# leejaeyong7/tiny-cuda-nn

Measured on AMD Instinct MI355X. Metric: training_step throughput (samples/s) HashGrid+64-wide FFMLP, batch=256k; % fp16-MFMA peak, higher is better.
Workload: dtype f16

## Files before the change

include/tcnn_amd.h:

```cpp
#ifndef TCNN_AMD_H
#define TCNN_AMD_H

#include <stddef.h>
#include <stdint.h>

#ifdef __cplusplus
extern "C" {
#endif

#define TCNN_OK 0
#define TCNN_ERROR 1

#define TCNN_PRECISION_FP32 0
#define TCNN_PRECISION_FP16 1

#define TCNN_GRADIENT_IGNORE 0
#define TCNN_GRADIENT_OVERWRITE 1
#define TCNN_GRADIENT_ACCUMULATE 2

#define TCNN_LAYOUT_SOA 0
#define TCNN_LAYOUT_AOS 1

#define TCNN_LOG_INFO 0
#define TCNN_LOG_DEBUG 1
// ... 91 lines not shown
int      tcnn_trainer_initialize_params(tcnn_trainer_t t);
int      tcnn_trainer_update_hyperparams(tcnn_trainer_t t, const char* json);
const char* tcnn_trainer_hyperparams(tcnn_trainer_t t);
int      tcnn_trainer_serialize(tcnn_trainer_t t, int serialize_optimizer, const void** out_bytes, size_t* out_size);
int      tcnn_trainer_deserialize(tcnn_trainer_t t, const void* bytes, size_t size);
const char* tcnn_trainer_network_hyperparams(tcnn_trainer_t t);
uint32_t tcnn_trainer_optimizer_step_count(tcnn_trainer_t t);
int  tcnn_trainer_profile_next_step(tcnn_trainer_t t);
int  tcnn_trainer_profile_collect(tcnn_trainer_t t, tcnn_stream_t stream, float* ms_per_piece , uint32_t* n_steps);
size_t tcnn_trainer_params_updated_in_flush(tcnn_trainer_t t);
size_t tcnn_trainer_image_preps(tcnn_trainer_t t);
size_t tcnn_trainer_scatter_wide_fallbacks(tcnn_trainer_t t);
size_t tcnn_trainer_optimizer_prologue_steps(tcnn_trainer_t t);
size_t tcnn_trainer_list_scatters(tcnn_trainer_t t);
size_t tcnn_module_list_scatters(tcnn_module_t m);
const char* tcnn_trainer_last_step_kernel(tcnn_trainer_t t);

int   tcnn_module_set_max_level(tcnn_module_t m, float max_level);
float tcnn_module_max_level(tcnn_module_t m);
int   tcnn_module_set_max_level_gpu(tcnn_module_t m, const float* per_sample);
int   tcnn_trainer_set_max_level(tcnn_trainer_t t, float max_level);
int   tcnn_trainer_set_max_level_gpu(tcnn_trainer_t t, const float* per_sample);
float tcnn_trainer_max_level(tcnn_trainer_t t);
int tcnn_train_ctx_keeps_weight_gradient_slabs(tcnn_trainer_t t, tcnn_train_ctx_t ctx);


int         tcnn_module_layer_sizes(tcnn_module_t m, uint32_t* rows_cols, size_t capacity, size_t* n_layers_out);
int         tcnn_optimizer_create(const char* optimizer_json, size_t n_params, const uint32_t* layer_sizes, size_t n_layers, tcnn_optimizer_t* out);
void        tcnn_optimizer_destroy(tcnn_optimizer_t o);
int         tcnn_optimizer_step(tcnn_optimizer_t o, tcnn_stream_t stream, float loss_scale, float* params_full_precision, void* params_half,
// ... 17 lines not shown
```

tiny-cuda-nn_amd/csrc/capi.cpp:

```cpp
#include "../../include/tcnn_amd.h"

#include "model.h"

#include <mutex>
#include <string>

using namespace tcnn_amd;

namespace {
thread_local std::string g_last_error;
tcnn_amd::Switches g_switches;
std::mutex g_switches_mutex;

bool env_is(const char* name, char c) {
	const char* e = getenv(name);
	return e && e[0] == c;
}
int env_01(const char* name) {
	const char* e = getenv(name);
	return (e && (e[0] == '0' || e[0] == '1')) ? e[0] - '0' : -1;
}

template <typename F>
int guarded(F&& f) {
// ... 61 lines not shown
	w.fused_step = !env_is("TCNN_AMD_FUSED_STEP", '0');
	w.side_jobs = !env_is("TCNN_AMD_SIDE_JOBS", '0');
	w.live_image = !env_is("TCNN_AMD_LIVE_IMAGE", '0');
	w.adam_steps32 = env_is("TCNN_AMD_ADAM_STEPS32", '1');
#ifdef TCNN_AMD_DEV
	w.adam_in_flush = env_is("TCNN_AMD_ADAM_IN_FLUSH", '1');
#endif
	w.adam_in_reduce = !env_is("TCNN_AMD_ADAM_IN_REDUCE", '0');
	w.adam_prologue = !env_is("TCNN_AMD_ADAM_PROLOGUE", '0');
	w.adam_prologue_refused = env_is("TCNN_AMD_ADAM_PROLOGUE", 'r');
	w.mlp_r32 = !env_is("TCNN_AMD_MLP_R32", '0');
	w.mlp_r32a = env_01("TCNN_AMD_MLP_R32A");
	w.mlp_regs = !env_is("TCNN_AMD_MLP_REGS", '0');
	w.mlp_fast = !env_is("TCNN_AMD_MLP_FAST", '0');
	if (const char* e = getenv("TCNN_AMD_MLP_PRIO")) w.mlp_prio = (uint32_t)atoi(e);
	w.mlp_layerwise = env_is("TCNN_AMD_MLP_LAYERWISE", '1');
	std::lock_guard<std::mutex> lock{g_switches_mutex};
	g_switches = w;
}
}

extern "C" {

const char* tcnn_last_error(void) { return g_last_error.c_str(); }
const char* tcnn_version(void) { return "tcnn_amd 0.1 (gfx950)"; }

uint32_t tcnn_batch_size_granularity(void) { return BATCH_SIZE_GRANULARITY; }

int tcnn_device(int* device_out) {
	return guarded([&] { HIP_CHECK_THROW(hipGetDevice(device_out)); });
// ... 266 lines not shown
		Trainer& tr = *t->trainer;
		tr.inference_mixed_precision((hipStream_t)stream, n, make_view(input, tr.model().input_width(), n, input_layout), output_half, use_inference_params != 0);
	});
}

size_t tcnn_trainer_n_params(tcnn_trainer_t t) { return t->trainer->n_params(); }
size_t tcnn_trainer_params_updated_in_flush(tcnn_trainer_t t) { return t->trainer->params_updated_in_flush(); }
size_t tcnn_trainer_image_preps(tcnn_trainer_t t) { return t->trainer->image_preps(); }
size_t tcnn_trainer_optimizer_prologue_steps(tcnn_trainer_t t) {
	try { return (size_t)t->trainer->prologue_steps(); } catch (const std::exception& e) { g_last_error = e.what(); return (size_t)-1; }
}
size_t tcnn_trainer_scatter_wide_fallbacks(tcnn_trainer_t t) {
	try { return (size_t)t->trainer->scatter_wide_fallbacks(); } catch (const std::exception& e) { g_last_error = e.what(); return (size_t)-1; }
}
size_t tcnn_trainer_list_scatters(tcnn_trainer_t t) { return (size_t)t->trainer->list_scatters(); }
const char* tcnn_trainer_last_step_kernel(tcnn_trainer_t t) { return t->trainer->last_step_kernel(); }
int tcnn_trainer_set_max_level(tcnn_trainer_t t, float max_level) {
	return guarded([&] {
		CHECK_THROW(t && t->trainer);
		if (!t->trainer->model().set_max_level(max_level)) no_grid(t->trainer->model());
	});
}
int tcnn_trainer_set_max_level_gpu(tcnn_trainer_t t, const float* per_sample) {
	return guarded([&] {
		CHECK_THROW(t && t->trainer);
		if (!t->trainer->model().set_max_level_gpu(per_sample)) no_grid(t->trainer->model());
	});
}
float tcnn_trainer_max_level(tcnn_trainer_t t) {
	float v = std::numeric_limits<float>::quiet_NaN();
// ... 192 lines not shown
```

tiny-cuda-nn_amd/csrc/k_grid_planes.hip:

```cpp
#include "grid_device.h"
#include "mlp_side_jobs.h"

#include <algorithm>
#include <cstdio>
#include <cstdlib>
#include <vector>

namespace tcnn_amd {
namespace {

constexpr int FP_THREADS = 128;
#ifndef TCNN_FP_LIST_THREADS
#define TCNN_FP_LIST_THREADS 256
#endif
constexpr int FP_LIST_THREADS = TCNN_FP_LIST_THREADS;

constexpr int FP_MAX_CHUNKS = GRID_FILTER_MAX_CHUNKS;
constexpr int FP_PER_LANE = FP_MAX_CHUNKS / 64;

template <int D, int F, int FP_SPT, bool LISTS>
__global__ void __launch_bounds__(LISTS ? FP_LIST_THREADS : FP_THREADS) k_grid_fwd_planes(
	const GridMeta* __restrict__ meta, const uint32_t* __restrict__ work, const uint32_t max_items, const uint32_t blocks_per_xcd, const uint32_t n, const MatView x,
	const half_t* __restrict__ grid, half_t* __restrict__ out, unsigned long long* __restrict__ bits, const MlpPrepJob prep, const GridHitLists lists
) {
// ... 327 lines not shown
	static const uint32_t dev_forced = getenv("TCNN_AMD_FWD_SPT") ? (uint32_t)atoi(getenv("TCNN_AMD_FWD_SPT")) : 0u;
	forced = dev_forced;
#endif
	if (max_scatter_chunks(meta) > (uint32_t)FP_MAX_CHUNKS) return 2u;
	if (forced == 8 || forced == 4 || forced == 2) return forced;
	if (meta.n_pos_dims == 3 && grid_scatter_prefers_lists(meta)) return 2u;
	return 4u;
}

bool grid_planes_supported(const GridMeta& meta, uint32_t n) {
	const uint32_t F = meta.n_features_per_level;
	return (F == 2 || F == 4 || F == 8) && (meta.n_pos_dims == 2 || meta.n_pos_dims == 3) && meta.n_levels < 256 && n % 64 == 0 && n > 0 &&
	       div_round_up(n, FP_THREADS * grid_planes_spt(meta)) < (1u << 24);
}

void grid_planes_plan(const GridMeta& meta, uint32_t n, bool hit_lists, std::vector<uint32_t>& work, uint32_t& max_items, uint32_t& blocks_per_xcd) {
	const uint32_t threads = hit_lists ? FP_LIST_THREADS : FP_THREADS;
	const uint32_t items_per_level = div_round_up(n, threads * grid_planes_spt(meta));
	float coarse_cost = 0.6f;
#ifdef TCNN_AMD_DEV
	if (const char* e = getenv("TCNN_AMD_FWD_COARSE_COST")) coarse_cost = (float)atof(e);
#endif
	std::vector<float> cost(meta.n_levels);
	double total = 0;
	for (uint32_t l = 0; l < meta.n_levels; ++l) {
		const size_t bytes = (size_t)meta.levels[l].size * meta.n_features_per_level * 2;
		cost[l] = bytes > (256u << 10) ? 1.0f : coarse_cost;
		total += (double)cost[l] * items_per_level;
	}
	uint32_t dbg_lo = 0, dbg_hi = meta.n_levels;
#ifdef TCNN_AMD_DEV
	if (const char* e = getenv("TCNN_AMD_FWD_LEVELS")) sscanf(e, "%u,%u", &dbg_lo, &dbg_hi);
#endif
	(void)total;
	size_t wide_bytes = (size_t)4 << 20;
#ifdef TCNN_AMD_DEV
	if (const char* e = getenv("TCNN_AMD_FWD_WIDE_MB")) wide_bytes = (size_t)std::max(atoi(e), 0) << 20;
#endif
	auto is_wide = [&](uint32_t l) { return wide_bytes > 0 && (size_t)meta.levels[l].size * meta.n_features_per_level * 2 > wide_bytes; };
	double narrow_total = 0;
	for (uint32_t l = 0; l < meta.n_levels; ++l) if (l >= dbg_lo && l <= dbg_hi && !is_wide(l)) narrow_total += (double)cost[l] * items_per_level;
	std::vector<std::vector<uint32_t>> runs(8);
	double acc = 0;
	for (uint32_t l = 0; l < meta.n_levels; ++l) {
		if (l < dbg_lo || l > dbg_hi || is_wide(l)) continue;
		for (uint32_t i = 0; i < items_per_level; ++i) {
			const uint32_t bin = std::min<uint32_t>((uint32_t)((acc + 0.5 * cost[l]) * 8.0 / narrow_total), 7u);
			runs[bin].push_back(l << 24 | i);
			acc += cost[l];
		}
	}
	{
		size_t longest = 0;
		for (auto& r : runs) longest = std::max(longest, r.size());
		uint32_t next = 0;
		for (uint32_t l = 0; l < meta.n_levels; ++l) {
			if (l < dbg_lo || l > dbg_hi || !is_wide(l)) continue;
			for (uint32_t i = 0; i < items_per_level; ++i) {
				size_t best = next % 8;
				for (size_t b = 0; b < 8; ++b) if (runs[b].size() < runs[best].size()) best = b;
				runs[best].push_back(l << 24 | i);
				++next;
			}
		}
		(void)longest;
	}
	max_items = 0;
	for (auto& r : runs) max_items = std::max<uint32_t>(max_items, (uint32_t)r.size());
	work.assign(8 + (size_t)8 * max_items, 0xffffffffu);
	for (uint32_t b = 0; b < 8; ++b) {
		work[b] = (uint32_t)runs[b].size();
		std::copy(runs[b].begin(), runs[b].end(), work.begin() + 8 + (size_t)b * max_items);
	}
	blocks_per_xcd = std::max(1u, std::min(256u * FP_THREADS / threads, max_items));
#ifdef TCNN_AMD_DEV
	if (const char* e = getenv("TCNN_AMD_FWD_BLOCKS_PER_XCD")) blocks_per_xcd = std::max(1, atoi(e));
#endif
}

void grid_forward_planes(hipStream_t stream, const GridMeta& meta, const GridMeta* dev_meta, const uint32_t* dev_work, uint32_t max_items, uint32_t blocks_per_xcd, uint32_t n,
                         MatView x, const void* grid, void* out_planes, uint64_t* chunk_bits, const MlpPrepJob* prep_job, const GridHitLists* hit_lists) {
	CHECK_THROW(grid_planes_supported(meta, n));
	CHECK_THROW(!hit_lists || (hit_lists->elems && hit_lists->heads && hit_lists->stragglers && hit_lists->counts && n <= grid_hit_max_samples(meta) &&
	                           hit_lists->item_samples == grid_hit_item_samples(meta) && hit_lists->n_items == div_round_up(n, hit_lists->item_samples) &&
	                           hit_lists->sidx && hit_lists->item_capacity >= (hit_lists->item_samples << (meta.n_pos_dims - 1)) && hit_lists->item_capacity % 8 == 0));
	const uint32_t F = meta.n_features_per_level;
#define TCNN_PLANES_F(D, SPT) \
	switch (F) { \
		case 2: return launch_planes<D, 2, SPT>(stream, dev_meta, dev_work, max_items, blocks_per_xcd, n, x, grid, out_planes, chunk_bits, prep_job, hit_lists); \
		case 4: return launch_planes<D, 4, SPT>(stream, dev_meta, dev_work, max_items, blocks_per_xcd, n, x, grid, out_planes, chunk_bits, prep_job, hit_lists); \
		default: return launch_planes<D, 8, SPT>(stream, dev_meta, dev_work, max_items, blocks_per_xcd, n, x, grid, out_planes, chunk_bits, prep_job, hit_lists); \
	}
// ... 60 lines not shown
```

tiny-cuda-nn_amd/csrc/model.h:

```cpp
#pragma once

#include "json_lite.h"
#include "tcnn_common.h"
#include "mlp_side_jobs.h"

#include <algorithm>
#include <cctype>
#include <cstdio>
#include <cmath>
#include <cstring>
#include <functional>
#include <limits>
#include <map>
#include <memory>
#include <mutex>
#include <numeric>
#include <random>
#include <unordered_map>
#include <vector>

namespace tcnn_amd {

struct LogSink {
	void (*callback)(int, const char*, void*) = nullptr;
// ... 198 lines not shown
	virtual EncodingContext forward(hipStream_t stream, uint32_t n, MatView x, const void* params, void* out, bool prepare_input_gradients, bool prepare_param_gradients) = 0;
	virtual void backward(hipStream_t stream, const EncodingContext& ctx, uint32_t n, MatView x, const void* dL_dy, MatViewMut* dL_dx, const void* params, void* grads, GradientMode mode, bool dy_planes) = 0;
	virtual void backward_backward_input(hipStream_t stream, const EncodingContext& ctx, uint32_t n, MatView x, MatView dL_ddLdx, const void* dL_dy, void* dL_ddLdy,
	                                     MatViewMut* dL_dx, const void* params, void* grads, GradientMode mode) {
		throw std::runtime_error{"DifferentiableObject::backward_backward_input_impl: not implemented error"};
	}
	virtual bool has_second_order() const { return false; }
	virtual bool second_order_reads_dL_dy() const { return true; }
	virtual uint32_t level_plane_features(bool need_dL_dx, GradientMode mode) const { return 0; }
	virtual bool as_identity(float& scale, float& offset) const { return false; }
	virtual uint32_t as_oneblob() const { return 0; }
	virtual bool scatter_records_usable(MatView x) const { return false; }
	virtual uint32_t scatter_record_planes() const { return 0; }
	virtual uint64_t scatter_wide_fallbacks() { return 0; }
	virtual uint64_t list_scatters() const { return 0; }
	virtual uint32_t forward_plane_features(uint32_t n) { return 0; }
	virtual EncodingContext forward_planes(hipStream_t stream, uint32_t n, MatView x, const void* params, void* out_planes, bool prepare_param_gradients,
	                                       const MlpPrepJob* prep_job = nullptr) {
		throw std::runtime_error{"Encoding: level-plane output is not available"};
	}
	virtual Json hyperparams() const = 0;
	bool fp32() const { return m_fp32; }
	virtual bool set_max_level(float max_level) { return false; }
	virtual bool set_max_level_gpu(const float* per_sample) { return false; }
	virtual bool get_max_level(float& max_level, const float*& per_sample) const { return false; }
protected:
	explicit Encoding(bool fp32) : m_fp32{fp32} {}
	bool m_fp32;
	uint32_t m_n_to_pad = 0;
};
// ... 147 lines not shown
			ctx.chunk_mask = ArenaBuf{stream, (size_t)m_meta.n_levels * grid_scatter_max_chunks() * (n / 64) * sizeof(uint64_t)};
			ctx.n = n;
			grid_mask_to_bits(stream, m_meta, dev_meta(), n, mask.as<uint64_t>(), ctx.chunk_mask.as<uint64_t>());
		}
		return ctx;
	}

	static bool use_planes() { return switches().grid_planes; }
	uint32_t forward_plane_features(uint32_t n) override {
		return (!m_fp32 && use_planes() && m_n_to_pad % m_meta.n_features_per_level == 0 && grid_planes_supported(m_meta, n)) ? m_meta.n_features_per_level : 0;
	}

	struct PlanesPlan {
		DeviceBuf dev_work;
		uint32_t max_items = 0, blocks_per_xcd = 0;
	};
	PlanesPlan& planes_plan(uint32_t n_, bool hit_lists) {
		const uint32_t n = n_ | (hit_lists ? 0x80000000u : 0u);
		auto it = m_planes_plans.find(n);
		if (it != m_planes_plans.end()) return *it->second;
		auto plan = std::make_unique<PlanesPlan>();
		std::vector<uint32_t> work;
		grid_planes_plan(m_meta, n_, hit_lists, work, plan->max_items, plan->blocks_per_xcd);
		plan->dev_work.resize(work.size() * sizeof(uint32_t));
		HIP_CHECK_THROW(hipMemcpy(plan->dev_work.data(), work.data(), work.size() * sizeof(uint32_t), hipMemcpyHostToDevice));
		return *(m_planes_plans[n] = std::move(plan));
	}

	EncodingContext forward_planes(hipStream_t stream, uint32_t n, MatView x, const void* params, void* out_planes, bool prepare_param_gradients,
	                               const MlpPrepJob* prep_job = nullptr) override {
		EncodingContext ctx;
		CHECK_THROW(forward_plane_features(n) > 0);
		const bool want_filter = prepare_param_gradients && lds_scatter_usable();
		const bool want_lists = want_filter && hit_lists_usable(n);
		if (want_lists) {
			HitCounters& hc = hit_counters(stream);
			GridHitLists& hl = ctx.hit_lists;
			hl.item_samples = grid_hit_item_samples(m_meta);
// ... 10 lines not shown
			hl.stragglers = (uint32_t*)((char*)ctx.hit_elems.data() + elems_bytes + sidx_bytes + heads_bytes);
			hl.counts = hc.sets[hc.next].as<uint32_t>();
			hl.zero_counts = hc.sets[hc.next ^ 1].as<uint32_t>();
			hc.next ^= 1;
#ifdef TCNN_AMD_DEV
			if (const char* e = getenv("TCNN_AMD_FWD_LISTS_DEV")) hl.dev_flags = (uint32_t)atoi(e);
#endif
			ctx.hit_generation = ++hc.generation;
			ctx.hit_stream = (const void*)stream;
			ctx.n = n;
		} else if (want_filter) {
			ctx.chunk_mask = ArenaBuf{stream, (size_t)m_meta.n_levels * grid_scatter_max_chunks() * (n / 64) * sizeof(uint64_t)};
			ctx.n = n;
		}
		PlanesPlan& plan = planes_plan(n, want_lists);
		grid_forward_planes(stream, m_meta, dev_meta(), plan.dev_work.as<uint32_t>(), plan.max_items, plan.blocks_per_xcd, n, x, params, out_planes, ctx.chunk_mask.as<uint64_t>(), prep_job,
		                    want_lists ? &ctx.hit_lists : nullptr);
		if (m_n_to_pad) HIP_CHECK_THROW(hipMemsetAsync((uint16_t*)out_planes + (size_t)n * m_n_features, 0, (size_t)n * m_n_to_pad * sizeof(uint16_t), stream));
		if (max_level_forward_active()) {
			const uint32_t F = m_meta.n_features_per_level;
			zero_levels(stream, 2, n, F, F, (uint64_t)n * F, out_planes, false);
		}
		return ctx;
	}

	void backward(hipStream_t stream, const EncodingContext& ctx, uint32_t n, MatView x, const void* dL_dy, MatViewMut* dL_dx, const void* params, void* grads, GradientMode mode, bool dy_planes) override {
		if ((!dL_dx && mode == GradientMode::Ignore) || n == 0) return;
		const uint32_t l_bwd = m_max_level_gpu ? m_meta.n_levels : levels_on(true);
		if (!m_max_level_gpu && l_bwd == m_meta.n_levels) return backward_all_levels(stream, ctx, n, x, dL_dy, dL_dx, params, grads, mode, dy_planes);
		if (m_max_level_gpu) {
// ... 271 lines not shown
		hc->fallbacks.memset(0);
		return *(m_hit_counters[(const void*)stream] = std::move(hc));
	}
public:
	uint64_t scatter_wide_fallbacks() override {
		uint64_t total = 0;
		for (auto& kv : m_hit_counters) {
			uint32_t v = 0;
			HIP_CHECK_THROW(hipMemcpy(&v, kv.second->fallbacks.data(), sizeof(v), hipMemcpyDeviceToHost));
			total += v;
		}
		return total;
	}

	uint64_t list_scatters() const override { return m_list_scatters; }

	bool set_max_level(float max_level) override { m_max_level = max_level; return true; }
	bool set_max_level_gpu(const float* per_sample) override { m_max_level_gpu = per_sample; return true; }
	bool get_max_level(float& max_level, const float*& per_sample) const override {
		max_level = m_max_level;
		per_sample = m_max_level_gpu;
		return true;
	}

	uint32_t levels_on(bool gradient_rule) const {
		const volatile float m = (m_max_level * (float)m_n_features) / (float)m_meta.n_features_per_level;
		const volatile float threshold = m + 1e-3f;
		for (uint32_t l = 0; l < m_meta.n_levels; ++l) {
			if (gradient_rule ? (float)l > threshold : (float)l >= threshold) return l;
		}
// ... 47 lines not shown
		j["hash"] = hashes[m_meta.hash_type];
		if (m_meta.grid_type == (uint32_t)GridType::Hash) j["log2_hashmap_size"] = m_log2_hashmap_size;
		return j;
	}

private:
	GridMeta m_meta;
	DeviceBuf m_dev_meta;
	std::map<std::pair<uint32_t, const void*>, std::unique_ptr<ScatterPlan>> m_scatter_plans;
	std::map<const void*, std::unique_ptr<HitCounters>> m_hit_counters;
	std::map<std::pair<uint32_t, const void*>, std::unique_ptr<ListsPlan>> m_lists_plans;
	std::map<uint32_t, std::unique_ptr<PlanesPlan>> m_planes_plans;
	bool m_scatter_levels_ok = true;
	bool m_any_binned = false;
	uint64_t m_list_scatters = 0;
	float m_max_level = 1000.f;
	const float* m_max_level_gpu = nullptr;
	std::vector<uint32_t> m_resolutions;
	uint32_t m_n_features, m_log2_hashmap_size, m_base_resolution, m_n_entries;
	float m_per_level_scale;
	bool m_stochastic_interpolation;
	size_t m_n_params;
};

class OneBlobEncoding : public Encoding {
public:
	OneBlobEncoding(uint32_t n_bins, uint32_t n_dims_to_encode, bool fp32) : Encoding{fp32}, m_n_bins{n_bins}, m_n_dims{n_dims_to_encode} {
		if ((n_bins & (n_bins - 1)) != 0 || n_bins == 0) throw std::runtime_error{"Number of bins must be a power of 2"};
	}
	uint32_t input_width() const override { return m_n_dims; }
// ... 534 lines not shown
private:
	enum class Reduction { Concatenation, Sum, Product };
	uint32_t reduction_width() const {
		for (const auto& e : m_nested) {
			if (e->padded_output_width() != e->output_width()) {
				throw std::runtime_error{"CompositeEncoding: a Sum / Product reduction needs nested encodings whose output width (" + std::to_string(e->output_width()) +
				                         ") is a multiple of the required alignment (padded to " + std::to_string(e->padded_output_width()) + ")"};
			}
		}
		return m_nested.front()->padded_output_width();
	}
public:
	uint64_t list_scatters() const override {
		uint64_t total = 0;
		for (const auto& e : m_nested) total += e->list_scatters();
		return total;
	}
	bool set_max_level(float max_level) override {
		bool any = false;
		for (auto& e : m_nested) any |= e->set_max_level(max_level);
		return any;
	}
	bool set_max_level_gpu(const float* per_sample) override {
		bool any = false;
		for (auto& e : m_nested) any |= e->set_max_level_gpu(per_sample);
		return any;
	}
	bool get_max_level(float& max_level, const float*& per_sample) const override {
		for (const auto& e : m_nested) {
			if (e->get_max_level(max_level, per_sample)) return true;
// ... 486 lines not shown
struct ModelContext {
	virtual ~ModelContext() {}
};

class Model {
public:
	virtual ~Model() {}
	virtual uint32_t input_width() const = 0;
	virtual uint32_t output_width() const = 0;
	virtual uint32_t padded_output_width() const = 0;
	virtual size_t n_params() const = 0;
	virtual Precision precision() const = 0;
	virtual std::vector<std::pair<uint32_t, uint32_t>> layer_sizes() const = 0;
	virtual void initialize_params(Pcg32& rng, float* params_full_precision, float scale) = 0;
	virtual uint64_t list_scatters() const { return 0; }
	virtual Encoding* input_encoding() { return nullptr; }
	bool set_max_level(float max_level) { Encoding* e = input_encoding(); return e && e->set_max_level(max_level); }
	bool set_max_level_gpu(const float* per_sample) { Encoding* e = input_encoding(); return e && e->set_max_level_gpu(per_sample); }
	bool get_max_level(float& max_level, const float*& per_sample) { Encoding* e = input_encoding(); return e && e->get_max_level(max_level, per_sample); }
	virtual void inference(hipStream_t stream, uint32_t n, MatView input, void* output, const void* params) = 0;
	virtual void inference_f32(hipStream_t stream, uint32_t n, MatView input, MatViewMut output, const void* params) {
		check_batch(n);
		if (n == 0) return;
		const uint32_t pw = padded_output_width();
		ArenaBuf tmp{stream, (size_t)n * pw * (precision() == Precision::Fp32 ? 4 : 2)};
		inference(stream, n, input, tmp.data(), params);
		trim_and_cast(stream, precision() == Precision::Fp32, n, pw, output_width(), tmp.data(), output);
	}
	virtual std::unique_ptr<ModelContext> forward(hipStream_t stream, uint32_t n, MatView input, void* output, const void* params, bool prepare_input_gradients) = 0;
	virtual void backward(hipStream_t stream, const ModelContext& ctx, uint32_t n, MatView input, const void* output, const void* dL_doutput,
// ... 238 lines not shown
		                     enc_grads ? GradientMode::Accumulate : GradientMode::Ignore, false);
		if (dL_dinput) add_input_gradient(stream, n, m_encoding->input_width(), MatView{dx_view.data, dx_view.stride_sample, dx_view.stride_dim}, *dL_dinput);
	}

	static bool use_fused_step() { return switches().fused_step; }
	static bool side_jobs_enabled() { return switches().side_jobs; }
	bool fused_step_supported(uint32_t n) const { return use_fused_step() && !m_network->layerwise() && mlp_train_any_kernel(m_network->desc(), n); }
	bool optimizer_rides_on_reduce() const { return m_encoding->n_params() == 0; }
	static bool live_image_enabled() { return switches().live_image; }
	bool live_image_kept() const { return m_live_image_kept; }
	void invalidate_live_image() { m_network->invalidate_live_image(); }
	size_t image_preps() const { return m_image_preps; }
	const char* last_train_kernel() const { return m_last_train_kernel; }
	uint64_t scatter_wide_fallbacks() { return m_encoding->scatter_wide_fallbacks(); }
	uint64_t list_scatters() const override { return m_encoding->list_scatters(); }
	bool context_keeps_slabs(const ModelContext& c) const { const Ctx* x = dynamic_cast<const Ctx*>(&c); return x && (bool)x->slabs_kept; }
	bool fused_compact_context_supported(uint32_t n) const {
		if (m_network->layerwise()) return false;
		const bool ok = use_fused_step() && mlp_train_compact_context(m_network->desc(), n) && m_network->padded_output_width() == 16;
		if (!ok && use_fused_step() && n > (1u << 22) && mlp_train_compact_context(m_network->desc(), 1u << 22)) {
			static bool told = false;
			if (!told) {
				told = true;
				const std::string msg = "training_step: batches of more than 4194304 rows run the general fused MLP kernel (several times slower for this network); split the batch to stay on the fast path";
				log_message(TCNN_LOG_WARNING, msg);
				fprintf(stderr, "tcnn_amd warning: %s\n", msg.c_str());
			}
		}
		return ok;
	}
// ... 172 lines not shown
};

class EncodingModel : public Model {
public:
	EncodingModel(uint32_t n_dims_to_encode, const Json& encoding, Precision precision) : m_precision{precision} {
		m_encoding = create_encoding(n_dims_to_encode, encoding, 0, precision == Precision::Fp32);
	}
	uint32_t input_width() const override { return m_encoding->input_width(); }
	uint32_t output_width() const override { return m_encoding->padded_output_width(); }
	uint32_t padded_output_width() const override { return m_encoding->padded_output_width(); }
	size_t n_params() const override { return m_encoding->n_params(); }
	Precision precision() const override { return m_precision; }
	std::vector<std::pair<uint32_t, uint32_t>> layer_sizes() const override { return {}; }
	void initialize_params(Pcg32& rng, float* params_full_precision, float scale) override { m_encoding->initialize_params(rng, params_full_precision, scale); }
	uint64_t list_scatters() const override { return m_encoding->list_scatters(); }
	Encoding* input_encoding() override { return m_encoding.get(); }

	struct Ctx : public ModelContext {
		EncodingContext encoding_ctx;
	};
	void inference(hipStream_t stream, uint32_t n, MatView input, void* output, const void* params) override {
		check_batch(n);
		m_encoding->forward(stream, n, input, params, output, false, false);
	}
	std::unique_ptr<ModelContext> forward(hipStream_t stream, uint32_t n, MatView input, void* output, const void* params, bool prepare_input_gradients) override {
		check_batch(n);
		auto ctx = std::make_unique<Ctx>();
		ctx->encoding_ctx = m_encoding->forward(stream, n, input, params, output, prepare_input_gradients, true);
		return ctx;
	}
// ... 1109 lines not shown
		j["loss"] = l;
		return j;
	}

	NetworkWithInputEncoding& model() { return *m_model; }
	Optimizer& optimizer() { return *m_optimizer; }
	StepProfile& profile() { return m_profile; }
	void* params_inference() const { void* custom = m_optimizer->custom_weights(); return custom ? custom : m_params.data(); }
	size_t n_params() const { return m_model->n_params(); }
	float* params_full_precision() { expose_params(); return m_params_fp.as<float>(); }
	void* params() { expose_params(); return m_params.data(); }
	const void* params_unexposed() const { return m_params.data(); }
	size_t image_preps() const { return m_model->image_preps(); }
	uint64_t scatter_wide_fallbacks() { return m_model->scatter_wide_fallbacks(); }
	uint64_t list_scatters() const { return m_model->list_scatters(); }
	size_t prologue_steps() const { return m_prologue_steps; }
	const char* last_step_kernel() const { return m_last_step_kernel; }
	void* param_gradients() const { return m_grads.data(); }

private:
	std::unique_ptr<NetworkWithInputEncoding> m_model;
	std::unique_ptr<Optimizer> m_optimizer;
	LossType m_loss;
	Pcg32 m_rng;
	DeviceBuf m_params_fp, m_params, m_grads, m_scalar;
	StepProfile m_profile;
	size_t m_params_updated_in_flush = 0;
	const char* m_last_step_kernel = "";
	bool m_params_exposed = false;
	void expose_params() {
// ... 7 lines not shown
```

tiny-cuda-nn_amd/csrc/tcnn_common.h:

```cpp
#pragma once

#include <hip/hip_runtime.h>

#include <cstddef>
#include <cstdint>
#include <stdexcept>
#include <string>
#include <vector>

namespace tcnn_amd {

enum class Activation : uint32_t { None = 0, ReLU = 1, LeakyReLU = 2, Exponential = 3, Sine = 4, Sigmoid = 5, Squareplus = 6, Softplus = 7, Tanh = 8 };
enum class GridType : uint32_t { Hash = 0, Dense = 1, Tiled = 2 };
enum class HashType : uint32_t { Prime = 0, CoherentPrime = 1, ReversedPrime = 2, Rng = 3 };
enum class InterpolationType : uint32_t { Nearest = 0, Linear = 1, Smoothstep = 2 };
enum class LossType : uint32_t { L2 = 0, RelativeL2 = 1, L1 = 2, RelativeL1 = 3, Mape = 4, Smape = 5, CrossEntropy = 6, Variance = 7, RelativeL2Luminance = 8 };
enum class Precision : uint32_t { Fp32 = 0, Fp16 = 1 };
enum class GradientPrecision : uint32_t { Fp32 = 0, Fp16 = 1 };
enum class GradientMode : uint32_t { Ignore = 0, Overwrite = 1, Accumulate = 2 };

constexpr uint32_t BATCH_SIZE_GRANULARITY = 256;
constexpr float LOSS_SCALE_FP16 = 128.0f;
constexpr uint32_t MAX_N_LEVELS = 128;
constexpr uint32_t MAX_MLP_LAYERS = 16;
// ... 16 lines not shown
	int scatter_lists = -1;
	bool scatter_wide = false;
	bool fused_step = true;
	bool side_jobs = true;
	bool live_image = true;
	bool adam_steps32 = false;
	bool adam_in_flush = false;
	bool adam_in_reduce = true;
	bool adam_prologue = true;
	bool adam_prologue_refused = false;
	bool mlp_r32 = true;
	int mlp_r32a = -1;
	bool mlp_regs = true;
	bool mlp_fast = true;
	uint32_t mlp_prio = 1;
	bool mlp_layerwise = false;
};
Switches switches();
void switches_reload();
inline uint32_t next_multiple(uint32_t v, uint32_t d) { return div_round_up(v, d) * d; }

struct GridLevel {
	uint32_t offset;
	uint32_t size;
	float    scale;
	uint32_t hashed;
	uint32_t stride[4];
	uint32_t size_mask;
	uint32_t scatter_per_chunk;
	uint32_t scatter_shift;
// ... 18 lines not shown
	uint32_t stride_dim;
};
struct MatViewMut {
	float* data;
	uint32_t stride_sample;
	uint32_t stride_dim;
};

void grid_forward(hipStream_t stream, const GridMeta& meta, const GridMeta* dev_meta, bool fp32, uint32_t n, MatView x, const void* grid, void* out, uint32_t out_stride, float* dy_dx,
                  uint64_t* chunk_mask);
bool grid_planes_supported(const GridMeta& meta, uint32_t n);
bool grid_planes_to_rows_supported(const GridMeta& meta, uint32_t n, uint32_t width);
void grid_planes_to_rows(hipStream_t stream, const GridMeta& meta, uint32_t n, uint32_t width, const void* planes, void* rows, uint32_t row_stride);
void grid_rows_to_planes(hipStream_t stream, const GridMeta& meta, uint32_t n, uint32_t width, const void* rows, uint32_t row_stride, void* planes);
uint32_t grid_planes_spt(const GridMeta& meta);
void grid_planes_plan(const GridMeta& meta, uint32_t n, bool hit_lists, std::vector<uint32_t>& work, uint32_t& max_items, uint32_t& blocks_per_xcd);
struct MlpPrepJob;
inline constexpr uint32_t grid_hit_mask_shift(uint32_t n_pos_dims) { return 32u - (1u << n_pos_dims); }
constexpr uint32_t GRID_HIT_COUNT_STRIDE = 64;
constexpr uint32_t GRID_HIT_HEADS = 65;
constexpr uint32_t GRID_HIT_WORDS = 2;
struct GridHitLists {
	uint32_t* elems = nullptr;
	uint16_t* sidx = nullptr;
	uint32_t* heads = nullptr;
	uint32_t* stragglers = nullptr;
	uint32_t* counts = nullptr;
	uint32_t* zero_counts = nullptr;
	uint32_t n_items = 0, item_samples = 0, item_capacity = 0, straggler_capacity = 0;
	uint32_t dev_flags = 0;
};
// ... 268 lines not shown
```

tiny-cuda-nn_amd/tinycudann/_C.py:

```python
import ctypes as C
import json
import os

_PKG = os.path.dirname(os.path.dirname(os.path.abspath(__file__)))
LIB_PATH = os.path.join(_PKG, "libtcnn_amd.so")
if os.environ.get("TCNN_AMD_LIB"):
    LIB_PATH = os.path.abspath(os.environ["TCNN_AMD_LIB"])

if not os.path.exists(LIB_PATH):
    raise ImportError(
        f"{LIB_PATH} not found: the HIP extension has not been built. Run `python tiny-cuda-nn_amd/build.py` "
        "(or __graft_entry__.build()). There is no CPU fallback."
    )

import torch

lib = C.CDLL(LIB_PATH)

_hip = None


def hip_runtime():
    global _hip
    if _hip is None:
# ... 71 lines not shown
    "tcnn_trainer_params": (_vp, [_vp]),
    "tcnn_trainer_params_inference": (_vp, [_vp]),
    "tcnn_trainer_param_gradients": (_vp, [_vp]),
    "tcnn_trainer_set_params_full_precision": (_int, [_vp, _vp, _sz, _int]),
    "tcnn_trainer_set_params": (_int, [_vp, _vp, _sz, _int]),
    "tcnn_trainer_initialize_params": (_int, [_vp]),
    "tcnn_trainer_update_hyperparams": (_int, [_vp, _cp]),
    "tcnn_trainer_hyperparams": (_cp, [_vp]),
    "tcnn_trainer_network_hyperparams": (_cp, [_vp]),
    "tcnn_trainer_optimizer_step_count": (_u32, [_vp]),
    "tcnn_trainer_params_updated_in_flush": (C.c_size_t, [_vp]),
    "tcnn_trainer_image_preps": (C.c_size_t, [_vp]),
    "tcnn_trainer_scatter_wide_fallbacks": (C.c_size_t, [_vp]),
    "tcnn_trainer_optimizer_prologue_steps": (C.c_size_t, [_vp]),
    "tcnn_trainer_list_scatters": (C.c_size_t, [_vp]),
    "tcnn_trainer_last_step_kernel": (_cp, [_vp]),
    "tcnn_trainer_set_max_level": (_int, [_vp, _f32]),
    "tcnn_trainer_set_max_level_gpu": (_int, [_vp, _vp]),
    "tcnn_trainer_max_level": (_f32, [_vp]),
    "tcnn_train_ctx_keeps_weight_gradient_slabs": (C.c_int, [_vp, _vp]),
    "tcnn_trainer_profile_next_step": (_int, [_vp]),
    "tcnn_trainer_profile_collect": (_int, [_vp, _vp, C.POINTER(C.c_float), C.POINTER(_u32)]),
    "tcnn_trainer_serialize": (_int, [_vp, _int, _pp, C.POINTER(_sz)]),
    "tcnn_trainer_deserialize": (_int, [_vp, _vp, _sz]),
    "tcnn_module_layer_sizes": (_int, [_vp, C.POINTER(_u32), _sz, C.POINTER(_sz)]),
    "tcnn_optimizer_create": (_int, [_cp, _sz, C.POINTER(_u32), _sz, _pp]),
    "tcnn_optimizer_destroy": (None, [_vp]),
    "tcnn_optimizer_step": (_int, [_vp, _vp, _f32, _vp, _vp, _vp, _int]),
    "tcnn_optimizer_step_count": (_u32, [_vp]),
    "tcnn_optimizer_n_params": (_sz, [_vp]),
# ... 59 lines not shown
```

tiny-cuda-nn_amd/tinycudann/native.py:

```python
import ctypes as C
import json

import torch

from . import _C

LAYOUT_SOA, LAYOUT_AOS = 0, 1
GRADIENT_IGNORE, GRADIENT_OVERWRITE, GRADIENT_ACCUMULATE = 0, 1, 2


def _ptr(t):
    return None if t is None else t.data_ptr()


def _stream(stream=None):
    if stream is None:
        return torch.cuda.current_stream().cuda_stream
    return stream.cuda_stream if hasattr(stream, "cuda_stream") else stream


class ForwardContext:

    def __init__(self, handle, n, padded_out):
        self._h = handle
# ... 58 lines not shown
    def profile_next_step(self):
        _C.check(_C.lib.tcnn_trainer_profile_next_step(self._h))

    def params_updated_in_flush(self):
        return int(_C.lib.tcnn_trainer_params_updated_in_flush(self._h))

    def image_preps(self):
        return int(_C.lib.tcnn_trainer_image_preps(self._h))

    def optimizer_prologue_steps(self):
        return int(_C.lib.tcnn_trainer_optimizer_prologue_steps(self._h))

    def list_scatters(self):
        return int(_C.lib.tcnn_trainer_list_scatters(self._h))

    def last_step_kernel(self):
        return _C.lib.tcnn_trainer_last_step_kernel(self._h).decode()

    def context_keeps_slabs(self, ctx):
        return bool(_C.lib.tcnn_train_ctx_keeps_weight_gradient_slabs(self._h, ctx._h))

    def scatter_wide_fallbacks(self):
        return int(_C.lib.tcnn_trainer_scatter_wide_fallbacks(self._h))

    def profile_collect(self, stream=None):
        ms = (C.c_float * 4)()
        n = C.c_uint32()
        _C.check(_C.lib.tcnn_trainer_profile_collect(self._h, _stream(stream), ms, C.byref(n)))
        k = max(n.value, 1)
        return {name: ms[i] / k for i, name in enumerate(self.PROFILE_PIECES)}, n.value
# ... 126 lines not shown
```

Before: 1.384 billion.

## Interleave small cache-resident grid levels among large levels in forward plane scheduling

The forward hash-grid plane planner can now pull out levels small enough to be cache-resident (up to 64KB). Instead of binning them into the XCD runs by cost, it interleaves them through the runs using a low-discrepancy (golden-ratio) sequence. Interleaving cheap, compute-bound work items among memory-bound large-level items is meant to overlap latency and balance the per-XCD runs. A counter of mixed forwards is exposed through the C and Python APIs. The new path is on by default behind TCNN_AMD_FWD_MIX and changes which items run together, which risks L2 locality for the large levels.

```diff
diff --git a/include/tcnn_amd.h b/include/tcnn_amd.h
--- a/include/tcnn_amd.h
+++ b/include/tcnn_amd.h
@@ -129,6 +129,7 @@
 size_t tcnn_trainer_optimizer_prologue_steps(tcnn_trainer_t t);
 size_t tcnn_trainer_list_scatters(tcnn_trainer_t t);
 size_t tcnn_module_list_scatters(tcnn_module_t m);
+size_t tcnn_trainer_mixed_forwards(tcnn_trainer_t t);
 const char* tcnn_trainer_last_step_kernel(tcnn_trainer_t t);
 
 int   tcnn_module_set_max_level(tcnn_module_t m, float max_level);
diff --git a/tiny-cuda-nn_amd/csrc/capi.cpp b/tiny-cuda-nn_amd/csrc/capi.cpp
--- a/tiny-cuda-nn_amd/csrc/capi.cpp
+++ b/tiny-cuda-nn_amd/csrc/capi.cpp
@@ -99,6 +99,7 @@
 	w.mlp_regs = !env_is("TCNN_AMD_MLP_REGS", '0');
 	w.mlp_fast = !env_is("TCNN_AMD_MLP_FAST", '0');
 	if (const char* e = getenv("TCNN_AMD_MLP_PRIO")) w.mlp_prio = (uint32_t)atoi(e);
+	w.fwd_mix = !env_is("TCNN_AMD_FWD_MIX", '0');
 	w.mlp_layerwise = env_is("TCNN_AMD_MLP_LAYERWISE", '1');
 	std::lock_guard<std::mutex> lock{g_switches_mutex};
 	g_switches = w;
@@ -395,6 +396,7 @@
 	try { return (size_t)t->trainer->scatter_wide_fallbacks(); } catch (const std::exception& e) { g_last_error = e.what(); return (size_t)-1; }
 }
 size_t tcnn_trainer_list_scatters(tcnn_trainer_t t) { return (size_t)t->trainer->list_scatters(); }
+size_t tcnn_trainer_mixed_forwards(tcnn_trainer_t t) { return (size_t)t->trainer->mixed_forwards(); }
 const char* tcnn_trainer_last_step_kernel(tcnn_trainer_t t) { return t->trainer->last_step_kernel(); }
 int tcnn_trainer_set_max_level(tcnn_trainer_t t, float max_level) {
 	return guarded([&] {
diff --git a/tiny-cuda-nn_amd/csrc/k_grid_planes.hip b/tiny-cuda-nn_amd/csrc/k_grid_planes.hip
--- a/tiny-cuda-nn_amd/csrc/k_grid_planes.hip
+++ b/tiny-cuda-nn_amd/csrc/k_grid_planes.hip
@@ -2,6 +2,7 @@
 #include "mlp_side_jobs.h"
 
 #include <algorithm>
+#include <cmath>
 #include <cstdio>
 #include <cstdlib>
 #include <vector>
@@ -365,48 +366,89 @@
 	       div_round_up(n, FP_THREADS * grid_planes_spt(meta)) < (1u << 24);
 }
 
-void grid_planes_plan(const GridMeta& meta, uint32_t n, bool hit_lists, std::vector<uint32_t>& work, uint32_t& max_items, uint32_t& blocks_per_xcd) {
+constexpr size_t FP_FREE_BYTES = 64u << 10, FP_L2_BYTES = 256u << 10;
+bool grid_planes_plan(const GridMeta& meta, uint32_t n, bool hit_lists, bool mix, std::vector<uint32_t>& work, uint32_t& max_items, uint32_t& blocks_per_xcd) {
 	const uint32_t threads = hit_lists ? FP_LIST_THREADS : FP_THREADS;
 	const uint32_t items_per_level = div_round_up(n, threads * grid_planes_spt(meta));
 	float coarse_cost = 0.6f;
+	size_t free_bytes = FP_FREE_BYTES;
 #ifdef TCNN_AMD_DEV
 	if (const char* e = getenv("TCNN_AMD_FWD_COARSE_COST")) coarse_cost = (float)atof(e);
-#endif
+	if (const char* e = getenv("TCNN_AMD_FWD_FREE_KB")) free_bytes = (size_t)std::max(atoi(e), 0) << 10;
+#endif
+	auto level_bytes = [&](uint32_t l) { return (size_t)meta.levels[l].size * meta.n_features_per_level * 2; };
 	std::vector<float> cost(meta.n_levels);
-	double total = 0;
-	for (uint32_t l = 0; l < meta.n_levels; ++l) {
-		const size_t bytes = (size_t)meta.levels[l].size * meta.n_features_per_level * 2;
-		cost[l] = bytes > (256u << 10) ? 1.0f : coarse_cost;
-		total += (double)cost[l] * items_per_level;
-	}
+	for (uint32_t l = 0; l < meta.n_levels; ++l) cost[l] = level_bytes(l) > FP_L2_BYTES ? 1.0f : coarse_cost;
 	uint32_t dbg_lo = 0, dbg_hi = meta.n_levels;
 #ifdef TCNN_AMD_DEV
 	if (const char* e = getenv("TCNN_AMD_FWD_LEVELS")) sscanf(e, "%u,%u", &dbg_lo, &dbg_hi);
 #endif
-	(void)total;
 	size_t wide_bytes = (size_t)4 << 20;
 #ifdef TCNN_AMD_DEV
 	if (const char* e = getenv("TCNN_AMD_FWD_WIDE_MB")) wide_bytes = (size_t)std::max(atoi(e), 0) << 20;
 #endif
-	auto is_wide = [&](uint32_t l) { return wide_bytes > 0 && (size_t)meta.levels[l].size * meta.n_features_per_level * 2 > wide_bytes; };
+	auto is_wide = [&](uint32_t l) { return wide_bytes > 0 && level_bytes(l) > wide_bytes; };
+	auto in_plan = [&](uint32_t l) { return l >= dbg_lo && l <= dbg_hi; };
+	auto is_free = [&](uint32_t l) { return level_bytes(l) <= free_bytes; };
+	uint32_t n_free = 0, n_affine = 0, n_l2 = 0;
+	for (uint32_t l = 0; l < meta.n_levels; ++l) if (in_plan(l) && !is_wide(l)) { ++(is_free(l) ? n_free : n_affine); n_l2 += level_bytes(l) > FP_L2_BYTES; }
+	const bool mixed = mix && n_free > 0 && n_l2 > 0;
+	if (mixed) std::fill(cost.begin(), cost.end(), 1.0f);
 	double narrow_total = 0;
-	for (uint32_t l = 0; l < meta.n_levels; ++l) if (l >= dbg_lo && l <= dbg_hi && !is_wide(l)) narrow_total += (double)cost[l] * items_per_level;
+	for (uint32_t l = 0; l < meta.n_levels; ++l) if (in_plan(l) && !is_wide(l) && !(mixed && is_free(l))) narrow_total += (double)cost[l] * items_per_level;
 	std::vector<std::vector<uint32_t>> runs(8);
 	double acc = 0;
 	for (uint32_t l = 0; l < meta.n_levels; ++l) {
-		if (l < dbg_lo || l > dbg_hi || is_wide(l)) continue;
+		if (!in_plan(l) || is_wide(l) || (mixed && is_free(l))) continue;
 		for (uint32_t i = 0; i < items_per_level; ++i) {
 			const uint32_t bin = std::min<uint32_t>((uint32_t)((acc + 0.5 * cost[l]) * 8.0 / narrow_total), 7u);
 			runs[bin].push_back(l << 24 | i);
 			acc += cost[l];
 		}
 	}
+	const uint32_t full_blocks = 256u * FP_THREADS / threads;
+	uint32_t forced_blocks = 0;
+#ifdef TCNN_AMD_DEV
+	if (const char* e = getenv("TCNN_AMD_FWD_BLOCKS_PER_XCD")) forced_blocks = (uint32_t)std::max(1, atoi(e));
+#endif
+	if (mixed) {
+		std::vector<uint32_t> free_items;
+		for (uint32_t l = 0; l < meta.n_levels; ++l) {
+			if (!in_plan(l) || is_wide(l) || !is_free(l)) continue;
+			for (uint32_t i = 0; i < items_per_level; ++i) free_items.push_back(l << 24 | i);
+		}
+		const size_t per_run = free_items.size() / 8, odd = free_items.size() % 8;
+		std::vector<uint32_t> by_length{0, 1, 2, 3, 4, 5, 6, 7};
+		std::stable_sort(by_length.begin(), by_length.end(), [&](uint32_t a, uint32_t b) { return runs[a].size() < runs[b].size(); });
+		size_t share[8], longest = 0;
+		for (uint32_t b = 0; b < 8; ++b) share[b] = per_run;
+		for (size_t j = 0; j < odd; ++j) ++share[by_length[j]];
+		for (uint32_t b = 0; b < 8; ++b) longest = std::max(longest, runs[b].size() + share[b]);
+		size_t n_wide = 0;
+		for (uint32_t l = 0; l < meta.n_levels; ++l) if (in_plan(l) && is_wide(l)) n_wide += items_per_level;
+		if (n_wide) longest = std::max(longest, (size_t)div_round_up((uint32_t)(n_wide + ((size_t)n_free + n_affine) * items_per_level), 8u));
+		const uint32_t walk = forced_blocks ? forced_blocks : std::max<uint32_t>(1u, std::min<uint32_t>(full_blocks, (uint32_t)longest));
+		size_t next_free = 0;
+		for (uint32_t b = 0; b < 8; ++b) {
+			const std::vector<uint32_t> affine = std::move(runs[b]);
+			std::vector<uint32_t>& run = runs[b];
+			run.clear();
+			size_t left_a = affine.size(), left_f = share[b];
+			uint32_t free_in_a_row = 0;
+			for (size_t p = 0; left_a + left_f > 0; ++p) {
+				const double key = (double)(p % walk) * 0.6180339887498949 + (double)(p / walk) * 0.4142135623730951;
+				bool take_free = left_f > 0 && (key - std::floor(key)) * (double)(left_a + left_f) < (double)left_f;
+				if (left_a == 0) take_free = true;
+				else if (free_in_a_row + 1 >= walk) take_free = false;
+				if (take_free) { run.push_back(free_items[next_free++]); --left_f; ++free_in_a_row; }
+				else { run.push_back(affine[affine.size() - left_a]); --left_a; free_in_a_row = 0; }
+			}
+		}
+	}
 	{
-		size_t longest = 0;
-		for (auto& r : runs) longest = std::max(longest, r.size());
 		uint32_t next = 0;
 		for (uint32_t l = 0; l < meta.n_levels; ++l) {
-			if (l < dbg_lo || l > dbg_hi || !is_wide(l)) continue;
+			if (!in_plan(l) || !is_wide(l)) continue;
 			for (uint32_t i = 0; i < items_per_level; ++i) {
 				size_t best = next % 8;
 				for (size_t b = 0; b < 8; ++b) if (runs[b].size() < runs[best].size()) best = b;
@@ -414,7 +456,6 @@
 				++next;
 			}
 		}
-		(void)longest;
 	}
 	max_items = 0;
 	for (auto& r : runs) max_items = std::max<uint32_t>(max_items, (uint32_t)r.size());
@@ -423,10 +464,8 @@
 		work[b] = (uint32_t)runs[b].size();
 		std::copy(runs[b].begin(), runs[b].end(), work.begin() + 8 + (size_t)b * max_items);
 	}
-	blocks_per_xcd = std::max(1u, std::min(256u * FP_THREADS / threads, max_items));
-#ifdef TCNN_AMD_DEV
-	if (const char* e = getenv("TCNN_AMD_FWD_BLOCKS_PER_XCD")) blocks_per_xcd = std::max(1, atoi(e));
-#endif
+	blocks_per_xcd = forced_blocks ? forced_blocks : std::max(1u, std::min(full_blocks, max_items));
+	return mixed;
 }
 
 void grid_forward_planes(hipStream_t stream, const GridMeta& meta, const GridMeta* dev_meta, const uint32_t* dev_work, uint32_t max_items, uint32_t blocks_per_xcd, uint32_t n,
diff --git a/tiny-cuda-nn_amd/csrc/model.h b/tiny-cuda-nn_amd/csrc/model.h
--- a/tiny-cuda-nn_amd/csrc/model.h
+++ b/tiny-cuda-nn_amd/csrc/model.h
@@ -236,6 +236,7 @@
 	virtual uint32_t scatter_record_planes() const { return 0; }
 	virtual uint64_t scatter_wide_fallbacks() { return 0; }
 	virtual uint64_t list_scatters() const { return 0; }
+	virtual uint64_t mixed_forwards() const { return 0; }
 	virtual uint32_t forward_plane_features(uint32_t n) { return 0; }
 	virtual EncodingContext forward_planes(hipStream_t stream, uint32_t n, MatView x, const void* params, void* out_planes, bool prepare_param_gradients,
 	                                       const MlpPrepJob* prep_job = nullptr) {
@@ -413,14 +414,16 @@
 	struct PlanesPlan {
 		DeviceBuf dev_work;
 		uint32_t max_items = 0, blocks_per_xcd = 0;
+		bool mixed = false;
 	};
 	PlanesPlan& planes_plan(uint32_t n_, bool hit_lists) {
-		const uint32_t n = n_ | (hit_lists ? 0x80000000u : 0u);
+		const bool mix = switches().fwd_mix;
+		const uint32_t n = n_ | (hit_lists ? 0x80000000u : 0u) | (mix ? 0x40000000u : 0u);
 		auto it = m_planes_plans.find(n);
 		if (it != m_planes_plans.end()) return *it->second;
 		auto plan = std::make_unique<PlanesPlan>();
 		std::vector<uint32_t> work;
-		grid_planes_plan(m_meta, n_, hit_lists, work, plan->max_items, plan->blocks_per_xcd);
+		plan->mixed = grid_planes_plan(m_meta, n_, hit_lists, mix, work, plan->max_items, plan->blocks_per_xcd);
 		plan->dev_work.resize(work.size() * sizeof(uint32_t));
 		HIP_CHECK_THROW(hipMemcpy(plan->dev_work.data(), work.data(), work.size() * sizeof(uint32_t), hipMemcpyHostToDevice));
 		return *(m_planes_plans[n] = std::move(plan));
@@ -461,6 +464,7 @@
 			ctx.n = n;
 		}
 		PlanesPlan& plan = planes_plan(n, want_lists);
+		if (plan.mixed) ++m_mixed_forwards;
 		grid_forward_planes(stream, m_meta, dev_meta(), plan.dev_work.as<uint32_t>(), plan.max_items, plan.blocks_per_xcd, n, x, params, out_planes, ctx.chunk_mask.as<uint64_t>(), prep_job,
 		                    want_lists ? &ctx.hit_lists : nullptr);
 		if (m_n_to_pad) HIP_CHECK_THROW(hipMemsetAsync((uint16_t*)out_planes + (size_t)n * m_n_features, 0, (size_t)n * m_n_to_pad * sizeof(uint16_t), stream));
@@ -762,6 +766,7 @@
 	}
 
 	uint64_t list_scatters() const override { return m_list_scatters; }
+	uint64_t mixed_forwards() const override { return m_mixed_forwards; }
 
 	bool set_max_level(float max_level) override { m_max_level = max_level; return true; }
 	bool set_max_level_gpu(const float* per_sample) override { m_max_level_gpu = per_sample; return true; }
@@ -839,6 +844,7 @@
 	bool m_scatter_levels_ok = true;
 	bool m_any_binned = false;
 	uint64_t m_list_scatters = 0;
+	uint64_t m_mixed_forwards = 0;
 	float m_max_level = 1000.f;
 	const float* m_max_level_gpu = nullptr;
 	std::vector<uint32_t> m_resolutions;
@@ -1403,6 +1409,11 @@
 	uint64_t list_scatters() const override {
 		uint64_t total = 0;
 		for (const auto& e : m_nested) total += e->list_scatters();
+		return total;
+	}
+	uint64_t mixed_forwards() const override {
+		uint64_t total = 0;
+		for (const auto& e : m_nested) total += e->mixed_forwards();
 		return total;
 	}
 	bool set_max_level(float max_level) override {
@@ -1919,6 +1930,7 @@
 	virtual std::vector<std::pair<uint32_t, uint32_t>> layer_sizes() const = 0;
 	virtual void initialize_params(Pcg32& rng, float* params_full_precision, float scale) = 0;
 	virtual uint64_t list_scatters() const { return 0; }
+	virtual uint64_t mixed_forwards() const { return 0; }
 	virtual Encoding* input_encoding() { return nullptr; }
 	bool set_max_level(float max_level) { Encoding* e = input_encoding(); return e && e->set_max_level(max_level); }
 	bool set_max_level_gpu(const float* per_sample) { Encoding* e = input_encoding(); return e && e->set_max_level_gpu(per_sample); }
@@ -2187,6 +2199,7 @@
 	const char* last_train_kernel() const { return m_last_train_kernel; }
 	uint64_t scatter_wide_fallbacks() { return m_encoding->scatter_wide_fallbacks(); }
 	uint64_t list_scatters() const override { return m_encoding->list_scatters(); }
+	uint64_t mixed_forwards() const override { return m_encoding->mixed_forwards(); }
 	bool context_keeps_slabs(const ModelContext& c) const { const Ctx* x = dynamic_cast<const Ctx*>(&c); return x && (bool)x->slabs_kept; }
 	bool fused_compact_context_supported(uint32_t n) const {
 		if (m_network->layerwise()) return false;
@@ -2389,6 +2402,7 @@
 	std::vector<std::pair<uint32_t, uint32_t>> layer_sizes() const override { return {}; }
 	void initialize_params(Pcg32& rng, float* params_full_precision, float scale) override { m_encoding->initialize_params(rng, params_full_precision, scale); }
 	uint64_t list_scatters() const override { return m_encoding->list_scatters(); }
+	uint64_t mixed_forwards() const override { return m_encoding->mixed_forwards(); }
 	Encoding* input_encoding() override { return m_encoding.get(); }
 
 	struct Ctx : public ModelContext {
@@ -3528,6 +3542,7 @@
 	size_t image_preps() const { return m_model->image_preps(); }
 	uint64_t scatter_wide_fallbacks() { return m_model->scatter_wide_fallbacks(); }
 	uint64_t list_scatters() const { return m_model->list_scatters(); }
+	uint64_t mixed_forwards() const { return m_model->mixed_forwards(); }
 	size_t prologue_steps() const { return m_prologue_steps; }
 	const char* last_step_kernel() const { return m_last_step_kernel; }
 	void* param_gradients() const { return m_grads.data(); }
diff --git a/tiny-cuda-nn_amd/csrc/tcnn_common.h b/tiny-cuda-nn_amd/csrc/tcnn_common.h
--- a/tiny-cuda-nn_amd/csrc/tcnn_common.h
+++ b/tiny-cuda-nn_amd/csrc/tcnn_common.h
@@ -54,6 +54,7 @@
 	bool mlp_regs = true;
 	bool mlp_fast = true;
 	uint32_t mlp_prio = 1;
+	bool fwd_mix = true;
 	bool mlp_layerwise = false;
 };
 Switches switches();
@@ -102,7 +103,7 @@
 void grid_planes_to_rows(hipStream_t stream, const GridMeta& meta, uint32_t n, uint32_t width, const void* planes, void* rows, uint32_t row_stride);
 void grid_rows_to_planes(hipStream_t stream, const GridMeta& meta, uint32_t n, uint32_t width, const void* rows, uint32_t row_stride, void* planes);
 uint32_t grid_planes_spt(const GridMeta& meta);
-void grid_planes_plan(const GridMeta& meta, uint32_t n, bool hit_lists, std::vector<uint32_t>& work, uint32_t& max_items, uint32_t& blocks_per_xcd);
+bool grid_planes_plan(const GridMeta& meta, uint32_t n, bool hit_lists, bool mix, std::vector<uint32_t>& work, uint32_t& max_items, uint32_t& blocks_per_xcd);
 struct MlpPrepJob;
 inline constexpr uint32_t grid_hit_mask_shift(uint32_t n_pos_dims) { return 32u - (1u << n_pos_dims); }
 constexpr uint32_t GRID_HIT_COUNT_STRIDE = 64;
diff --git a/tiny-cuda-nn_amd/tinycudann/_C.py b/tiny-cuda-nn_amd/tinycudann/_C.py
--- a/tiny-cuda-nn_amd/tinycudann/_C.py
+++ b/tiny-cuda-nn_amd/tinycudann/_C.py
@@ -109,6 +109,7 @@
     "tcnn_trainer_scatter_wide_fallbacks": (C.c_size_t, [_vp]),
     "tcnn_trainer_optimizer_prologue_steps": (C.c_size_t, [_vp]),
     "tcnn_trainer_list_scatters": (C.c_size_t, [_vp]),
+    "tcnn_trainer_mixed_forwards": (C.c_size_t, [_vp]),
     "tcnn_trainer_last_step_kernel": (_cp, [_vp]),
     "tcnn_trainer_set_max_level": (_int, [_vp, _f32]),
     "tcnn_trainer_set_max_level_gpu": (_int, [_vp, _vp]),
diff --git a/tiny-cuda-nn_amd/tinycudann/native.py b/tiny-cuda-nn_amd/tinycudann/native.py
--- a/tiny-cuda-nn_amd/tinycudann/native.py
+++ b/tiny-cuda-nn_amd/tinycudann/native.py
@@ -96,6 +96,9 @@
     def list_scatters(self):
         return int(_C.lib.tcnn_trainer_list_scatters(self._h))
 
+    def mixed_forwards(self):
+        return int(_C.lib.tcnn_trainer_mixed_forwards(self._h))
+
     def last_step_kernel(self):
         return _C.lib.tcnn_trainer_last_step_kernel(self._h).decode()
 
```

New measurement: 1.369 billion. -1.1%, worse.
